# jac99/Egonn

Hardware: AMD Instinct MI355X
Metric: LiDAR scans/sec (descriptor extraction), 50k-pt clouds @ 0.1m voxel (higher is better)
Workload: dtype f32

## Files before the change

egonn_amd/_lib.py:

```python
from __future__ import annotations

import ctypes as C
import os
from typing import List, Optional, Sequence

import numpy as np
import torch

_HERE = os.path.dirname(os.path.abspath(__file__))
LIB_PATH = os.path.join(_HERE, "lib", "libegonn_hip.so")

QUANT_CARTESIAN, QUANT_POLAR = 0, 1
FLAG_DISABLE_GLOBAL, FLAG_DISABLE_LOCAL, FLAG_IGNORE_KP_REGRESSOR, FLAG_BF16 = 1, 2, 4, 8
FLAG_POOL_SPOC, FLAG_POOL_MAC = 16, 32
MINKFPN_SPLIT_TOPDOWN = 1
MINKFPN_BLOCKS = {'BasicBlock': 0, 'ECABasicBlock': 1}
MINKFPN_POOLING = {None: 0, 'GeM': 1, 'MAC': 2, 'SPoC': 3}

_P = C.c_void_p
_SIGS = [
    ("egonn_ctx_create", C.c_int, [C.POINTER(_P), C.c_int, C.c_int]),
    ("egonn_ctx_destroy", None, [_P]),
    ("egonn_last_error", C.c_char_p, []),
    ("egonn_debug_set_naive_conv", C.c_int, [_P, C.c_int]),
    ("egonn_debug_set_ksplit", C.c_int, [_P, C.c_int, C.c_int, C.c_int, C.c_int, C.c_int]),
    ("egonn_debug_set_resident", C.c_int, [_P, C.c_int, C.c_int]),
    ("egonn_debug_keep_level_features", C.c_int, [_P, C.c_int]),
    ("egonn_debug_set_trace", C.c_int, [_P]),
    ("egonn_prepare_maps", C.c_int, [_P, C.c_int, _P]),
    ("egonn_debug_rowgroup_tables", C.c_int, [_P, C.c_int, C.c_int, _P, _P, C.c_int64, C.POINTER(C.c_int64), _P]),
    ("egonn_debug_rowgroup_perm", C.c_int, [_P, C.c_int, C.c_int, _P, C.c_int64, C.POINTER(C.c_int64), _P]),
    ("egonn_debug_radix_sort_scratch_bytes", C.c_int64, [C.c_int64, C.c_int]),
    ("egonn_debug_radix_sort", C.c_int, [_P, _P, _P, _P, C.c_int64, C.c_int, _P, _P, C.c_int, C.c_int, C.c_int,
                                         C.POINTER(C.c_int32), _P, C.c_int64, _P]),
    ("egonn_debug_dense_group3", C.c_int, [_P, _P, _P, _P, _P, _P, _P]),
    ("egonn_debug_global_tail_scratch_bytes", C.c_int64, [C.c_int64]),
    ("egonn_debug_global_tail", C.c_int, [_P, _P, C.c_int, C.c_int64, _P, _P, _P, _P, _P, _P, C.c_int, C.c_int, _P, _P, _P, C.c_int64, _P]),
    ("egonn_voxelize", C.c_int, [_P, _P, C.POINTER(C.c_int64), C.c_int, C.c_int, C.POINTER(C.c_float), _P]),
    ("egonn_ctx_reserve", C.c_int, [_P, C.c_int64, C.c_int, C.POINTER(C.c_int64)]),
    ("egonn_voxelize_device", C.c_int, [_P, _P, C.c_int64, _P, C.c_int, C.c_int, C.POINTER(C.c_float), _P]),
    ("egonn_plan_status", C.c_int, [_P, _P]),
    ("egonn_ctx_set_exact_fp32", C.c_int, [_P, C.c_int]),
    ("egonn_ctx_set_operand_autoscale", C.c_int, [_P, C.c_int]),
    ("egonn_level_capacity", C.c_int, [_P, C.c_int, C.POINTER(C.c_int64)]),
    ("egonn_graph_begin", C.c_int, [_P]),
    ("egonn_graph_end", C.c_int, [_P, C.POINTER(_P)]),
    ("egonn_graph_launch", C.c_int, [_P, _P]),
    ("egonn_graph_destroy", None, [_P]),
    ("egonn_coords_set", C.c_int, [_P, _P, C.c_int64, C.c_int, _P]),
    ("egonn_level_count", C.c_int, [_P, C.c_int, C.POINTER(C.c_int64)]),
    ("egonn_level_batch_offsets", C.c_int, [_P, C.c_int, C.POINTER(C.c_int64)]),
    ("egonn_level_coords", C.c_int, [_P, C.c_int, _P, _P]),
    ("egonn_input_index", C.c_int, [_P, _P, _P]),
    ("egonn_conv", C.c_int, [_P, C.c_int, C.c_int, C.c_int, _P, C.c_int, _P, C.c_int, _P, _P, C.c_int, _P, _P]),
# ... 899 lines not shown
```

egonn_amd/csrc/coords.hip:

```cpp
#include "common.h"

#include <algorithm>
#include <stdarg.h>

namespace egonn {

static thread_local char g_err[1024] = "";
void set_error(const char* fmt, ...) {
  va_list ap;
  va_start(ap, fmt);
  vsnprintf(g_err, sizeof(g_err), fmt, ap);
  va_end(ap);
}
const char* last_error() { return g_err; }

const Switches& switches() {
  static const Switches sw = [] {
    auto on = [](const char* name) { return getenv(name) != nullptr; };
    auto num = [](const char* name, int unset) { const char* e = getenv(name); return e ? atoi(e) : unset; };
    const char* ds = getenv("EGONN_DEBUG_SYNC");
    return Switches{.debug_sync = ds && ds[0] == '1', .no_presplit = on("EGONN_NO_PRESPLIT"), .no_fused_down = on("EGONN_NO_FUSED_DOWN"),
                    .no_fused_lateral = on("EGONN_NO_FUSED_LATERAL"), .no_gated_k2s2 = on("EGONN_NO_GATED_K2S2"),
                    .no_fused_ghead = on("EGONN_NO_FUSED_GHEAD"), .no_fused_gtail = on("EGONN_NO_FUSED_GTAIL"),
                    .no_packed_laterals = on("EGONN_NO_PACKED_LATERALS"), .no_split_heads = on("EGONN_NO_SPLIT_HEADS"),
// ... 123 lines not shown
    vals[i] = (uint32_t)i;
  }
}

__global__ void coords_to_keys_kernel(const int32_t* __restrict__ c4, int64_t n, int cb, int Bmax,
                                      uint64_t* __restrict__ keys, uint32_t* __restrict__ vals,
                                      int32_t* __restrict__ flags) {
  const int64_t i = (int64_t)blockIdx.x * blockDim.x + threadIdx.x;
  if (i >= n) return;
  const int4 c = reinterpret_cast<const int4*>(c4)[i];
  uint64_t key;
  if (!encode_key(c.x, c.y, c.z, c.w, cb, key) || c.x >= Bmax) {
    atomicOr(flags, 1);
    key = ~0ull >> 1;
  }
  keys[i] = key;
  vals[i] = (uint32_t)i;
}

static constexpr int PYR_BLOCK = 256;
static constexpr int PYR_ROUNDS = 4;
static constexpr int PYR_TILE = PYR_BLOCK * PYR_ROUNDS;
static constexpr int NL = EGONN_MAX_LEVELS;

__device__ static inline int head_levels(const uint64_t* __restrict__ keys, int64_t i) {
  if (i == 0) return NL;
  const uint64_t d = keys[i] ^ keys[i - 1];
  if (d == 0) return 0;
  const int t = (63 - __clzll(d)) / 3;
  return (t >= NL - 1) ? NL : t + 1;
}

__device__ static inline int64_t clip_count(int64_t cap, const int64_t* __restrict__ n_dev) {
  if (!n_dev) return cap;
  const int64_t v = *n_dev;
  return v < cap ? v : cap;
}
__global__ __launch_bounds__(PYR_BLOCK) void pyramid_count_kernel(const uint64_t* __restrict__ keys, int64_t n_cap,
                                                                  const int64_t* __restrict__ n_dev,
                                                                  int32_t* __restrict__ tilecnt) {
  __shared__ int32_t cnt[PYR_BLOCK / 64][NL];
  const int64_t n = clip_count(n_cap, n_dev);
  const int tid = threadIdx.x, lane = tid & 63, wave = tid >> 6;
  const int64_t wbase = (int64_t)blockIdx.x * PYR_TILE + (int64_t)wave * 64 * PYR_ROUNDS;
  int32_t c[NL];
#pragma unroll
  for (int l = 0; l < NL; ++l) c[l] = 0;
  for (int r = 0; r < PYR_ROUNDS; ++r) {
    const int64_t i = wbase + r * 64 + lane;
    const int h = (i < n) ? head_levels(keys, i) : 0;
#pragma unroll
    for (int l = 0; l < NL; ++l) c[l] += __popcll(__ballot(h > l));
  }
  if (lane == 0) {
#pragma unroll
    for (int l = 0; l < NL; ++l) cnt[wave][l] = c[l];
  }
  __syncthreads();
  if (tid < NL) {
    int32_t s = 0;
    for (int w = 0; w < PYR_BLOCK / 64; ++w) s += cnt[w][tid];
    tilecnt[(int64_t)blockIdx.x * NL + tid] = s;
  }
}

struct PyramidOut {
  uint64_t* keys[NL];
  int32_t* parent[NL];
  int32_t* cstart[NL];
  int32_t* boff[EGONN_NUM_LEVELS];
  int32_t* perm0;
  int32_t* counts;
  int32_t* flags;
  int32_t cap[NL];
};

__global__ __launch_bounds__(PYR_BLOCK) void pyramid_apply_kernel(const uint64_t* __restrict__ keys,
                                                                  const uint32_t* __restrict__ vals, int64_t n_cap,
                                                                  const int64_t* __restrict__ n_dev,
                                                                  const int32_t* __restrict__ tilecnt, int ntiles,
                                                                  int cb, int B, PyramidOut out) {
  __shared__ int32_t red[PYR_BLOCK / 64][NL];
  const int64_t n = clip_count(n_cap, n_dev);
  __shared__ int32_t tilebase[NL];
  __shared__ int32_t wavecnt[PYR_BLOCK / 64][NL];
  const int tid = threadIdx.x, lane = tid & 63, wave = tid >> 6;
  const int tile = blockIdx.x;

  {
    int32_t p[NL];
#pragma unroll
    for (int l = 0; l < NL; ++l) p[l] = 0;
    for (int t = tid; t < tile; t += PYR_BLOCK) {
#pragma unroll
      for (int l = 0; l < NL; ++l) p[l] += tilecnt[(int64_t)t * NL + l];
    }
#pragma unroll
    for (int l = 0; l < NL; ++l) {
      int32_t v = p[l];
#pragma unroll
      for (int o = 32; o > 0; o >>= 1) v += __shfl_down(v, o, 64);
      if (lane == 0) red[wave][l] = v;
    }
    __syncthreads();
    if (tid < NL) {
      int32_t s = 0;
      for (int w = 0; w < PYR_BLOCK / 64; ++w) s += red[w][tid];
      tilebase[tid] = s;
    }
  }

  const int64_t wbase = (int64_t)tile * PYR_TILE + (int64_t)wave * 64 * PYR_ROUNDS;
  int hreg[PYR_ROUNDS];
  int32_t wc[NL];
#pragma unroll
  for (int l = 0; l < NL; ++l) wc[l] = 0;
#pragma unroll
  for (int r = 0; r < PYR_ROUNDS; ++r) {
    const int64_t i = wbase + r * 64 + lane;
    hreg[r] = (i < n) ? head_levels(keys, i) : 0;
#pragma unroll
    for (int l = 0; l < NL; ++l) wc[l] += __popcll(__ballot(hreg[r] > l));
  }
  if (lane == 0) {
#pragma unroll
    for (int l = 0; l < NL; ++l) wavecnt[wave][l] = wc[l];
  }
  __syncthreads();
  int32_t run[NL];
#pragma unroll
  for (int l = 0; l < NL; ++l) {
    int32_t s = tilebase[l];
    for (int w = 0; w < wave; ++w) s += wavecnt[w][l];
    run[l] = s;
  }

  const uint64_t lt = (lane == 0) ? 0ull : (~0ull >> (64 - lane));
  const int bshift = 3 * cb;
#pragma unroll
  for (int r = 0; r < PYR_ROUNDS; ++r) {
    const int64_t i = wbase + r * 64 + lane;
    const int h = hreg[r];
    const uint64_t key = (i < n) ? keys[i] : 0ull;
    int32_t excl[NL];
#pragma unroll
    for (int l = 0; l < NL; ++l) {
      const uint64_t m = __ballot(h > l);
      excl[l] = run[l] + __popcll(m & lt);
      run[l] += __popcll(m);
    }
    if (i < n && h > 0) {
      if (excl[0] < out.cap[0]) out.perm0[excl[0]] = (int32_t)vals[i];
#pragma unroll
      for (int l = 0; l < NL; ++l) {
        if (l < h && excl[l] < out.cap[l]) {
          out.keys[l][excl[l]] = key >> (3 * l);
          if (l >= 1) out.cstart[l][excl[l]] = min(excl[l - 1], out.cap[l - 1]);
          if (l + 1 < NL) {
            const int32_t g = (l + 1 < h) ? excl[l + 1] : excl[l + 1] - 1;
            out.parent[l][excl[l]] = min(g, out.cap[l + 1] - 1);
          }
        }
      }
      const int32_t b = (int32_t)(key >> bshift);
      const int32_t bprev = (i == 0) ? -1 : (int32_t)(keys[i - 1] >> bshift);
      if (b != bprev) {
        for (int32_t bb = bprev + 1; bb <= b && bb <= B; ++bb) {
#pragma unroll
          for (int l = 0; l < EGONN_NUM_LEVELS; ++l) out.boff[l][bb] = min(excl[l], out.cap[l]);
        }
      }
    }
    if (i == n - 1) {
      const int32_t blast = (int32_t)(key >> bshift);
#pragma unroll
      for (int l = 0; l < NL; ++l) {
        const int32_t total = excl[l] + (h > l ? 1 : 0);
        out.counts[l] = total;
        if (total > out.cap[l]) atomicOr(out.flags, 2);
        if (l >= 1) {
          const int32_t below = excl[l - 1] + (h > l - 1 ? 1 : 0);
          out.cstart[l][min(total, out.cap[l])] = min(below, out.cap[l - 1]);
        }
        if (l < EGONN_NUM_LEVELS) {
          for (int32_t bb = blast + 1; bb <= B; ++bb) out.boff[l][bb] = min(total, out.cap[l]);
        }
      }
      out.counts[NL] = blast + 1;
      out.counts[NL + 1] = (int32_t)n;
    }
  }
}

struct MaskArgs {
  const int32_t* cstartL[NL];
  const uint64_t* keys[NL];
  uint64_t* mask[NL];
  int32_t* bstart[NL];
  const int32_t* counts;
  int32_t prefix[NL + 1];
};

__device__ static inline int32_t level_rows(const int32_t* __restrict__ counts, int l, int32_t cap) {
  const int32_t v = counts[l];
  return v < cap ? v : cap;
}

__device__ static inline void block_mask_body(const MaskArgs& a, uint32_t vblock) {
  const int64_t t = (int64_t)vblock * 256 + threadIdx.x;
  if (t >= a.prefix[NL]) return;
  int L = 2;
  while (L < NL - 1 && t >= a.prefix[L + 1]) ++L;
  const int32_t j = (int32_t)(t - a.prefix[L]);
  if (j >= level_rows(a.counts, L, a.prefix[L + 1] - a.prefix[L])) return;
  const int32_t* cs1 = a.cstartL[L];
  const int32_t* cs2 = a.cstartL[L - 1];
  const int32_t s = cs2[cs1[j]];
  const int32_t e = cs2[cs1[j + 1]];
  const uint64_t* k = a.keys[L - 2];
  uint64_t m = 0;
  for (int32_t r = s; r < e; ++r) m |= 1ull << (k[r] & 63);
  a.mask[L][j] = m;
  a.bstart[L][j] = s;
}

__device__ static inline int32_t find_key(const uint64_t* __restrict__ keys, int32_t n, uint64_t q) {
  int32_t lo = 0, hi = n;
  while (lo < hi) {
    const int32_t mid = (lo + hi) >> 1;
    if (keys[mid] < q) lo = mid + 1; else hi = mid;
  }
  return (lo < n && keys[lo] == q) ? lo : -1;
}

__device__ static inline uint32_t bit_of_local(uint32_t lx, uint32_t ly, uint32_t lz) {
  return (lx & 1) | ((ly & 1) << 1) | ((lz & 1) << 2) | ((lx & 2) << 2) | ((ly & 2) << 3) | ((lz & 2) << 4);
}

__device__ static inline int32_t lookup_local(const uint64_t* nbm, const int32_t* nbs, int32_t nx, int32_t ny,
                                              int32_t nz) {
  const int32_t sx = (nx < 0) ? 0 : (nx > 3 ? 2 : 1);
  const int32_t sy = (ny < 0) ? 0 : (ny > 3 ? 2 : 1);
  const int32_t sz = (nz < 0) ? 0 : (nz > 3 ? 2 : 1);
  const int32_t slot = sx + 3 * sy + 9 * sz;
// ... 46 lines not shown
  const int32_t* badj;
  const uint64_t* bmask;
  const int32_t* bstart;
  int32_t* nbr;
  int32_t level, cap_blocks, cap_vox;
};
struct Blk27Args {
  const int32_t* badj;
  const uint64_t* bmask;
  const int32_t* bstart;
  int32_t cap2;
  uint64_t* t2m;
  int32_t* t2s;
};
struct Nbr27Pair {
  Nbr27Job job[2];
  const int32_t* counts;
  uint32_t split;
  uint32_t tail_at;
  Blk27Args blk;
};
__device__ static inline void blk27_body(const Blk27Args& b, const int32_t* __restrict__ counts, uint32_t vblock) {
  const int32_t t = (int32_t)(vblock * 256 + threadIdx.x);
  if (t >= level_rows(counts, 2, b.cap2) * 27) return;
  const int32_t a = b.badj[t];
  b.t2m[t] = a >= 0 ? b.bmask[a] : 0ull;
  b.t2s[t] = a >= 0 ? b.bstart[a] : 0;
}
__global__ __launch_bounds__(256) void nbr27_kernel(const Nbr27Pair a) {
  if (blockIdx.x >= a.tail_at) {
    blk27_body(a.blk, a.counts, blockIdx.x - a.tail_at);
    return;
  }
  const bool second = blockIdx.x >= a.split;
  const Nbr27Job& J = a.job[second ? 1 : 0];
  const uint64_t* __restrict__ vkeys = J.vkeys;
  const int32_t* __restrict__ badj = J.badj;
  const uint64_t* __restrict__ bmask = J.bmask;
  const int32_t* __restrict__ bstart = J.bstart;
  const int32_t* __restrict__ counts = a.counts;
  int32_t* __restrict__ nbr = J.nbr;
  const int level = J.level;
  const int32_t cap_blocks = J.cap_blocks, cap_vox = J.cap_vox;
  const uint32_t bid = second ? blockIdx.x - a.split : blockIdx.x;
  __shared__ uint64_t s_m[4][27];
  __shared__ int32_t s_s[4][27];
  const int lane = threadIdx.x & 63, wave = threadIdx.x >> 6;
  const int32_t j = (int32_t)bid * 4 + wave;
  const int32_t nblocks = level_rows(counts, level + 2, cap_blocks), nvox = level_rows(counts, level, cap_vox);
  if (j >= nblocks) return;
  const int32_t s = min(bstart[j], nvox);
  const int32_t e = min((j + 1 < nblocks) ? bstart[j + 1] : nvox, nvox);
  const int32_t idx = (lane < 27) ? badj[(int64_t)j * 27 + lane] : -1;
  const int32_t items = (e - s) * 27;
  uint64_t key0 = 0;
  if (lane < items) key0 = vkeys[s + lane / 27];
  if (lane < 27) {
    s_m[wave][lane] = idx >= 0 ? bmask[idx] : 0ull;
    s_s[wave][lane] = idx >= 0 ? bstart[idx] : 0;
  }
  __builtin_amdgcn_wave_barrier();
  __builtin_amdgcn_fence(__ATOMIC_ACQ_REL, "wavefront");
  for (int32_t t = lane; t < items; t += 64) {
    const int32_t v = t / 27, k = t - v * 27;
    const uint32_t lk = (uint32_t)((t == lane ? key0 : vkeys[s + v]) & 63);
    const int32_t lx = (lk & 1) | ((lk >> 2) & 2), ly = ((lk >> 1) & 1) | ((lk >> 3) & 2),
                  lz = ((lk >> 2) & 1) | ((lk >> 4) & 2);
    const int32_t nx = lx + (k % 3) - 1, ny = ly + (k / 3) % 3 - 1, nz = lz + k / 9 - 1;
    nbr[(int64_t)s * 27 + t] = lookup_local(s_m[wave], s_s[wave], nx, ny, nz);
  }
}

__global__ void count_valid_kernel(const int32_t* __restrict__ tbl, int64_t n, unsigned long long* __restrict__ out) {
  __shared__ int32_t red[4];
  int32_t c = 0;
  for (int64_t i = (int64_t)blockIdx.x * blockDim.x + threadIdx.x; i < n; i += (int64_t)gridDim.x * blockDim.x)
    c += (tbl[i] >= 0);
#pragma unroll
  for (int o = 32; o > 0; o >>= 1) c += __shfl_xor(c, o, 64);
  if ((threadIdx.x & 63) == 0) red[threadIdx.x >> 6] = c;
  __syncthreads();
  if (threadIdx.x == 0) atomicAdd(out, (unsigned long long)(red[0] + red[1] + red[2] + red[3]));
}
__global__ void count_k5_pairs_kernel(const uint64_t* __restrict__ vkeys, const int32_t* __restrict__ g0,
                                      const uint64_t* __restrict__ t2m, int32_t n, unsigned long long* __restrict__ out) {
  __shared__ int32_t red[4];
  int32_t c = 0;
  for (int32_t i = blockIdx.x * blockDim.x + threadIdx.x; i < n; i += gridDim.x * blockDim.x) {
    const uint32_t lk = (uint32_t)(vkeys[i] & 63);
    const int lx = (lk & 1) | ((lk >> 2) & 2), ly = ((lk >> 1) & 1) | ((lk >> 3) & 2), lz = ((lk >> 2) & 1) | ((lk >> 4) & 2);
    const uint64_t* m27 = t2m + (int64_t)g0[i] * 27;
    for (int k = 0; k < 125; ++k) {
// ... 42 lines not shown

__global__ void nbrT_kernel(const int32_t* __restrict__ parent, const uint64_t* __restrict__ keys,
                            const int32_t* __restrict__ counts, int32_t cap, int32_t* __restrict__ nbrT) {
  const int32_t c = blockIdx.x * blockDim.x + threadIdx.x;
  if (c >= level_rows(counts, 0, cap)) return;
  const int slot = (int)(keys[c] & 7);
  const int32_t p = parent[c];
  int32_t r[8];
#pragma unroll
  for (int q = 0; q < 8; ++q) r[q] = (q == slot) ? p : -1;
  int4* o = reinterpret_cast<int4*>(nbrT + (int64_t)c * 8);
  o[0] = make_int4(r[0], r[1], r[2], r[3]);
  o[1] = make_int4(r[4], r[5], r[6], r[7]);
}

struct Nbr8TArgs {
  const int32_t* cstart[EGONN_NUM_LEVELS];
  const uint64_t* ckeys[EGONN_NUM_LEVELS];
  const int32_t* parent[EGONN_NUM_LEVELS];
  const uint64_t* keys[EGONN_NUM_LEVELS];
  int32_t* nbr8[EGONN_NUM_LEVELS];
  int32_t* nbrT[EGONN_NUM_LEVELS];
  const int32_t* counts;
  int32_t prefix[EGONN_NUM_LEVELS + 1];
};
__device__ static inline void nbr8T_all_body(const Nbr8TArgs& a, uint32_t vblock) {
  const int64_t t = (int64_t)vblock * 256 + threadIdx.x;
  if (t >= a.prefix[EGONN_NUM_LEVELS]) return;
  int l = 1;
  while (l < EGONN_NUM_LEVELS - 1 && t >= a.prefix[l + 1]) ++l;
  const int32_t p = (int32_t)(t - a.prefix[l]);
  if (p >= level_rows(a.counts, l, a.prefix[l + 1] - a.prefix[l])) return;
  {
    int32_t r[8] = {-1, -1, -1, -1, -1, -1, -1, -1};
    const int32_t s = a.cstart[l][p], e = a.cstart[l][p + 1];
    const uint64_t* ck = a.ckeys[l];
    for (int32_t c = s; c < e; ++c) {
      const int slot = (int)(ck[c] & 7);
#pragma unroll
      for (int q = 0; q < 8; ++q)
        if (q == slot) r[q] = c;
    }
    int4* o = reinterpret_cast<int4*>(a.nbr8[l] + (int64_t)p * 8);
    o[0] = make_int4(r[0], r[1], r[2], r[3]);
    o[1] = make_int4(r[4], r[5], r[6], r[7]);
  }
  {
    const int slot = (int)(a.keys[l][p] & 7);
    const int32_t par = a.parent[l][p];
    int32_t r[8];
#pragma unroll
    for (int q = 0; q < 8; ++q) r[q] = (q == slot) ? par : -1;
    int4* o = reinterpret_cast<int4*>(a.nbrT[l] + (int64_t)p * 8);
    o[0] = make_int4(r[0], r[1], r[2], r[3]);
    o[1] = make_int4(r[4], r[5], r[6], r[7]);
  }
}

struct PlanTablesArgs {
  MaskArgs ma;
  Adj27Args adj;
  Adj27Args adj2;
  Nbr8TArgs na;
  const int32_t *parent0, *parent1;
  int32_t* g0;
  int32_t cap0;
  uint32_t b_mask, b_adj, b_adj2, b_gp, b_n8;
};
__global__ __launch_bounds__(256) void plan_tables_kernel(const PlanTablesArgs a) {
  uint32_t b = blockIdx.x;
  if (b < a.b_mask) { block_mask_body(a.ma, b); return; }
  b -= a.b_mask;
  if (b < a.b_adj) { adj27_search_body(a.adj, b); return; }
  b -= a.b_adj;
  if (b < a.b_adj2) { adj27_search_body(a.adj2, b); return; }
  b -= a.b_adj2;
  if (b < a.b_gp) {
    const int32_t i = (int32_t)(b * 256 + threadIdx.x);
    if (i < level_rows(a.ma.counts, 0, a.cap0)) a.g0[i] = a.parent1[a.parent0[i]];
    return;
  }
  b -= a.b_gp;
  nbr8T_all_body(a.na, b);
}

__global__ void decode_coords_kernel(const uint64_t* __restrict__ keys, int32_t n, int level, int cb,
                                     int32_t* __restrict__ out) {
  const int32_t i = blockIdx.x * blockDim.x + threadIdx.x;
  if (i >= n) return;
  const int cbL = cb - level;
  const uint64_t key = keys[i];
  const uint64_t mort = key & ((1ull << (3 * cbL)) - 1);
  const int32_t bias = 1 << (cb - 1);
  int4 o;
  o.x = (int32_t)(key >> (3 * cbL));
  o.y = ((int32_t)compact1by2(mort) << level) - bias;
  o.z = ((int32_t)compact1by2(mort >> 1) << level) - bias;
  o.w = ((int32_t)compact1by2(mort >> 2) << level) - bias;
  reinterpret_cast<int4*>(out)[i] = o;
}

static int batch_bits(int B) {
  int b = 0;
  while ((1 << b) < B) ++b;
  return b < 1 ? 1 : b;
}
// ... 98 lines not shown
  P.coord_bits = cb;
  P.n_input = n;
  P.cap_points = n;
  P.valid = true;
  P.exact = false;
  P.built_reserved = reserved;
  if (!reserved) {
    EGONN_TRY(plan_sync(ctx, stream));
    for (int l = 0; l < NL; ++l) P.cap[l] = P.lv[l].n;
  } else {
    for (int l = 0; l < NL; ++l) P.lv[l].n = P.cap[l];
  }
  P.valid = false;
  const int32_t* counts = ctx->dev_counts;

  PlanTablesArgs ta;
  MaskArgs& ma = ta.ma;
  int32_t pre = 0;
  for (int L = 0; L < NL; ++L) {
    ma.cstartL[L] = P.lv[L].cstart;
    ma.keys[L] = P.lv[L].keys;
    ma.mask[L] = nullptr;
    ma.bstart[L] = nullptr;
    ma.prefix[L] = 0;
  }
  ma.counts = counts;
  for (int L = 2; L < NL; ++L) {
    P.lv[L].mask = ma.mask[L] = A.alloc<uint64_t>(P.cap[L]);
    P.lv[L].bstart = ma.bstart[L] = A.alloc<int32_t>(P.cap[L]);
    EGONN_REQUIRE(ma.mask[L] && ma.bstart[L], EGONN_ERR_STATE, "plan arena too small");
    ma.prefix[L] = pre;
    pre += (int32_t)P.cap[L];
  }
  ma.prefix[NL] = pre;
  ta.b_mask = (unsigned)cdiv(pre, 256);
  for (int l = NL - 1; l >= 1; --l) {
    P.lv[l].nbr27 = A.alloc<int32_t>((size_t)P.cap[l] * 27);
    EGONN_REQUIRE(P.lv[l].nbr27, EGONN_ERR_STATE, "plan arena too small");
  }
  {
    Level& V = P.lv[NL - 2];
    Level& V1 = P.lv[NL - 1];
    const int32_t nv = (int32_t)P.cap[NL - 2], nv1 = (int32_t)P.cap[NL - 1];
    ta.adj = Adj27Args{V.keys, V1.keys, counts, NL - 2, NL - 1, cb - (NL - 2), cb - (NL - 1), nv, nv1, V.nbr27, V1.nbr27};
    ta.b_adj = (unsigned)cdiv(((int64_t)nv + nv1) * 27, 256);
  }
  const bool search67_ok = !switches().no_search67;
  const int search_from = (search67_ok && P.cap[NL - 4] <= 8192 && P.cap[NL - 3] <= 8192) ? NL - 4 : NL - 2;
  ta.b_adj2 = 0;
  ta.adj2 = ta.adj;
  if (search_from == NL - 4) {
    Level& V = P.lv[NL - 4];
    Level& V1 = P.lv[NL - 3];
    const int32_t nv = (int32_t)P.cap[NL - 4], nv1 = (int32_t)P.cap[NL - 3];
    ta.adj2 = Adj27Args{V.keys, V1.keys, counts, NL - 4, NL - 3, cb - (NL - 4), cb - (NL - 3), nv, nv1, V.nbr27, V1.nbr27};
    ta.b_adj2 = (unsigned)cdiv(((int64_t)nv + nv1) * 27, 256);
  }
  const int32_t n0 = (int32_t)P.cap[0], n2 = (int32_t)P.cap[2];
  {
    P.g0 = A.alloc<int32_t>(n0);
    P.t2m = A.alloc<uint64_t>((size_t)n2 * 27);
    P.t2s = A.alloc<int32_t>((size_t)n2 * 27);
    EGONN_REQUIRE(P.g0 && P.t2m && P.t2s, EGONN_ERR_STATE, "plan arena too small");
    ta.parent0 = P.lv[0].parent; ta.parent1 = P.lv[1].parent; ta.g0 = P.g0; ta.cap0 = n0;
    ta.b_gp = (unsigned)cdiv(n0, 256);
  }
  {
    Nbr8TArgs& na = ta.na;
    na.prefix[0] = na.prefix[1] = 0;
    na.counts = counts;
    for (int l = 1; l < EGONN_NUM_LEVELS; ++l) {
      Level& V = P.lv[l];
      const int32_t nv = (int32_t)P.cap[l];
      V.nbr8 = A.alloc<int32_t>((size_t)nv * 8);
      V.nbrT = A.alloc<int32_t>((size_t)nv * 8);
      EGONN_REQUIRE(V.nbr8 && V.nbrT, EGONN_ERR_STATE, "plan arena too small");
      na.cstart[l] = V.cstart;
      na.ckeys[l] = P.lv[l - 1].keys;
      na.parent[l] = V.parent;
      na.keys[l] = V.keys;
      na.nbr8[l] = V.nbr8;
      na.nbrT[l] = V.nbrT;
      na.prefix[l + 1] = na.prefix[l] + nv;
    }
    na.cstart[0] = nullptr; na.ckeys[0] = nullptr; na.parent[0] = nullptr; na.keys[0] = nullptr;
    na.nbr8[0] = nullptr; na.nbrT[0] = nullptr;
    ta.b_n8 = (unsigned)cdiv(na.prefix[EGONN_NUM_LEVELS], 256);
  }
  {
    const unsigned nb = ta.b_mask + ta.b_adj + ta.b_adj2 + ta.b_gp + ta.b_n8;
    if (nb > 0) hipLaunchKernelGGL(plan_tables_kernel, dim3(nb), dim3(256), 0, stream, ta);
  }

  Nbr27Pair pair;
  int npair = 0;
  pair.counts = counts;
  pair.split = 0;
  pair.tail_at = ~0u;
  pair.blk = Blk27Args{nullptr, nullptr, nullptr, 0, nullptr, nullptr};
  bool blk_done = false;
  auto flush = [&](bool last) {
    if (npair == 0 && !(last && !blk_done && n0 > 0)) return;
    if (npair == 1) pair.job[1] = pair.job[0];
    const unsigned g0 = npair >= 1 ? pair.split : 0u, g1 = npair == 2 ? (unsigned)cdiv(pair.job[1].cap_blocks, 4) : 0u;
    if (npair == 0) { pair.split = 0; pair.job[0] = Nbr27Job{nullptr, nullptr, nullptr, nullptr, nullptr, 1, 0, 0}; pair.job[1] = pair.job[0]; }
    unsigned extra = 0;
    pair.tail_at = ~0u;
    if (last && !blk_done && n0 > 0) {
      pair.tail_at = g0 + g1;
      pair.blk = Blk27Args{P.lv[2].nbr27, P.lv[2].mask, P.lv[2].bstart, n2, P.t2m, P.t2s};
// ... 170 lines not shown
    ctx->reserve_cap[l] = c;
  }
  ctx->reserve_points = max_points;
  ctx->reserve_batch = B;
  EGONN_TRY(ctx->plan_arena.ensure(plan_arena_bytes(max_points, B)));
  EGONN_TRY(ctx->sort_arena.ensure(std::max(radix_sort_scratch_bytes(max_points), radix_sort_segments_scratch_bytes(max_points, B))));
  ctx->reserved = true;
  return EGONN_OK;
}

int plan_level_coords(Ctx* ctx, int level, int32_t* out, hipStream_t stream) {
  EGONN_REQUIRE(ctx->plan.valid, EGONN_ERR_STATE, "no coordinate plan (call egonn_voxelize / egonn_coords_set first)");
  EGONN_REQUIRE(level >= 0 && level < EGONN_MAX_LEVELS, EGONN_ERR_INVALID, "level %d out of range", level);
  EGONN_TRY(plan_sync(ctx, stream));
  const Level& L = ctx->plan.lv[level];
  if (L.n == 0) return EGONN_OK;
  hipLaunchKernelGGL(decode_coords_kernel, dim3((unsigned)cdiv(L.n, 256)), dim3(256), 0, stream, L.keys, (int32_t)L.n,
                     level, ctx->plan.coord_bits, out);
  HIP_CHECK(hipGetLastError());
  return EGONN_OK;
}

}
```

include/egonn_hip.h:

```cpp
#ifndef EGONN_HIP_H
#define EGONN_HIP_H

#include <stdint.h>

#ifdef __cplusplus
extern "C" {
#endif

typedef struct egonn_ctx egonn_ctx;
typedef struct egonn_model egonn_model;

enum { EGONN_QUANT_CARTESIAN = 0, EGONN_QUANT_POLAR = 1 };
enum { EGONN_STATUS_OK = 0, EGONN_STATUS_INVALID = 1, EGONN_STATUS_HIP = 2, EGONN_STATUS_RANGE = 3, EGONN_STATUS_STATE = 4,
       EGONN_STATUS_CAPACITY = 5,
       EGONN_STATUS_FP16_RANGE = 6 };
enum { EGONN_FLAG_DISABLE_GLOBAL = 1, EGONN_FLAG_DISABLE_LOCAL = 2, EGONN_FLAG_IGNORE_KP_REGRESSOR = 4,
       EGONN_FLAG_BF16 = 8,
       EGONN_FLAG_POOL_SPOC = 16, EGONN_FLAG_POOL_MAC = 32 };

int egonn_ctx_create(egonn_ctx** ctx, int device, int coord_bits);
void egonn_ctx_destroy(egonn_ctx* ctx);
const char* egonn_last_error(void);
int egonn_debug_set_naive_conv(egonn_ctx* ctx, int on);
int egonn_debug_set_ksplit(egonn_ctx* ctx, int map_class, int level, int kparts, int kw, int col_parts);
int egonn_debug_set_resident(egonn_ctx* ctx, int mask, int max_workgroups);
int egonn_debug_keep_level_features(egonn_ctx* ctx, int on);
int egonn_debug_set_trace(void* device_buffer);
int egonn_debug_rowgroup_tables(egonn_ctx* ctx, int map_kind, int level_out, uint32_t* gmask_out, int32_t* snbr_out,
                                int64_t capacity_groups, int64_t* n_groups, void* stream);
int egonn_debug_rowgroup_perm(egonn_ctx* ctx, int map_kind, int level_out, int32_t* perm_out, int64_t capacity_groups,
                              int64_t* n_groups, void* stream);
int64_t egonn_debug_radix_sort_scratch_bytes(int64_t n, int n_segments);
int egonn_debug_radix_sort(uint64_t* keys_in, uint32_t* vals_in, uint64_t* keys_out, uint32_t* vals_out, int64_t n, int nbits,
                           const int64_t* n_dev, const int64_t* seg_offsets, int n_segments, int idx_bits, int either_pair,
                           int32_t* result_pair, void* scratch, int64_t scratch_bytes, void* stream);
int egonn_debug_dense_group3(const float* const in[3], const int64_t rows_capacity[3], const int32_t* const n_dev[3],
                             const float* const weight[3], const float* const packed[3], float* const out[3], void* stream);
int64_t egonn_debug_global_tail_scratch_bytes(int64_t rows_capacity);
int egonn_debug_global_tail(const float* g5, const int32_t* row_offsets, int batch_size, int64_t rows_capacity, const int32_t* n_dev,
                            const float* w0, const float* b0, const float* w1, const float* b1, const float* p, int pooling, int form,
                            float* partial, float* out, void* scratch, int64_t scratch_bytes, void* stream);

int egonn_voxelize(egonn_ctx* ctx, const float* points, const int64_t* scan_offsets, int batch_size, int quant_mode,
                   const float* step, void* stream);
int egonn_ctx_reserve(egonn_ctx* ctx, int64_t max_points, int batch_size, const int64_t* level_capacity);
int egonn_voxelize_device(egonn_ctx* ctx, const float* points, int64_t n_rows, const int64_t* scan_offsets_dev,
                          int batch_size, int quant_mode, const float* step, void* stream);
int egonn_plan_status(egonn_ctx* ctx, void* stream);
int egonn_ctx_set_exact_fp32(egonn_ctx* ctx, int on);
int egonn_ctx_set_operand_autoscale(egonn_ctx* ctx, int on);
int egonn_level_capacity(egonn_ctx* ctx, int level, int64_t* capacity);
typedef struct egonn_graph egonn_graph;
int egonn_graph_begin(void* stream);
int egonn_graph_end(void* stream, egonn_graph** graph);
// ... 351 lines not shown
```

Measured before the change: 23410.

## Hoist loads ahead of dependent work in coordinate-pyramid and plan-table kernels

The pyramid apply kernel now loads its keys and values into registers up front and gets each previous key through a wave shuffle rather than a second global read. It also packs the head levels into 4-bit fields. The mask, nbr8T, blk27, nbr27 and plan-table kernels clamp their indices so global loads can issue before the bounds checks, with sched barriers to keep that order. Level dispatch now uses per-level workgroup offsets instead of a linear prefix search, and child scans are unrolled in batches of 8 loads. New debug APIs expose the plan arena and its tables, and the clamped speculative loads read some redundant data.

```diff
diff --git a/egonn_amd/_lib.py b/egonn_amd/_lib.py
--- a/egonn_amd/_lib.py
+++ b/egonn_amd/_lib.py
@@ -30,6 +30,8 @@
     ("egonn_prepare_maps", C.c_int, [_P, C.c_int, _P]),
     ("egonn_debug_rowgroup_tables", C.c_int, [_P, C.c_int, C.c_int, _P, _P, C.c_int64, C.POINTER(C.c_int64), _P]),
     ("egonn_debug_rowgroup_perm", C.c_int, [_P, C.c_int, C.c_int, _P, C.c_int64, C.POINTER(C.c_int64), _P]),
+    ("egonn_debug_plan_arena", C.c_int, [_P, _P, C.c_int64, C.c_int, C.POINTER(C.c_int64)]),
+    ("egonn_debug_plan_tables", C.c_int, [_P, C.POINTER(C.c_int64), C.c_int, C.POINTER(C.c_int)]),
     ("egonn_debug_radix_sort_scratch_bytes", C.c_int64, [C.c_int64, C.c_int]),
     ("egonn_debug_radix_sort", C.c_int, [_P, _P, _P, _P, C.c_int64, C.c_int, _P, _P, C.c_int, C.c_int, C.c_int,
                                          C.POINTER(C.c_int32), _P, C.c_int64, _P]),
diff --git a/egonn_amd/csrc/coords.hip b/egonn_amd/csrc/coords.hip
--- a/egonn_amd/csrc/coords.hip
+++ b/egonn_amd/csrc/coords.hip
@@ -1,4 +1,4 @@
-#include "common.h"
+#include "model.h"
 
 #include <algorithm>
 #include <stdarg.h>
@@ -169,13 +169,17 @@
 static constexpr int PYR_ROUNDS = 4;
 static constexpr int PYR_TILE = PYR_BLOCK * PYR_ROUNDS;
 static constexpr int NL = EGONN_MAX_LEVELS;
-
-__device__ static inline int head_levels(const uint64_t* __restrict__ keys, int64_t i) {
-  if (i == 0) return NL;
-  const uint64_t d = keys[i] ^ keys[i - 1];
+static_assert(NL <= 15, "pyramid_apply_kernel packs a head level into 4 bits");
+
+__device__ static inline int head_levels_of(uint64_t key, uint64_t prev, bool first) {
+  if (first) return NL;
+  const uint64_t d = key ^ prev;
   if (d == 0) return 0;
   const int t = (63 - __clzll(d)) / 3;
   return (t >= NL - 1) ? NL : t + 1;
+}
+__device__ static inline int head_levels(const uint64_t* __restrict__ keys, int64_t i) {
+  return i == 0 ? NL : head_levels_of(keys[i], keys[i - 1], false);
 }
 
 __device__ static inline int64_t clip_count(int64_t cap, const int64_t* __restrict__ n_dev) {
@@ -183,6 +187,28 @@
   const int64_t v = *n_dev;
   return v < cap ? v : cap;
 }
+
+struct PyrKeys {
+  uint64_t key[PYR_ROUNDS];
+  uint64_t front;
+};
+__device__ static inline PyrKeys pyramid_load_keys(const uint64_t* __restrict__ keys, int64_t n_cap, int64_t wbase, int lane) {
+  PyrKeys k;
+  const int64_t last = n_cap - 1;
+#pragma unroll
+  for (int r = 0; r < PYR_ROUNDS; ++r) {
+    const int64_t i = wbase + r * 64 + lane;
+    k.key[r] = keys[i < last ? i : last];
+  }
+  const int64_t f = wbase - 1 < last ? wbase - 1 : last;
+  k.front = keys[f > 0 ? f : 0];
+  return k;
+}
+__device__ static inline uint64_t pyramid_prev_key(uint64_t key, uint64_t carry, int lane) {
+  const uint64_t up = __shfl_up(key, 1, 64);
+  return lane == 0 ? carry : up;
+}
+
 __global__ __launch_bounds__(PYR_BLOCK) void pyramid_count_kernel(const uint64_t* __restrict__ keys, int64_t n_cap,
                                                                   const int64_t* __restrict__ n_dev,
                                                                   int32_t* __restrict__ tilecnt) {
@@ -228,11 +254,20 @@
                                                                   const int32_t* __restrict__ tilecnt, int ntiles,
                                                                   int cb, int B, PyramidOut out) {
   __shared__ int32_t red[PYR_BLOCK / 64][NL];
-  const int64_t n = clip_count(n_cap, n_dev);
   __shared__ int32_t tilebase[NL];
   __shared__ int32_t wavecnt[PYR_BLOCK / 64][NL];
   const int tid = threadIdx.x, lane = tid & 63, wave = tid >> 6;
   const int tile = blockIdx.x;
+  const int64_t wbase = (int64_t)tile * PYR_TILE + (int64_t)wave * 64 * PYR_ROUNDS;
+  const PyrKeys k = pyramid_load_keys(keys, n_cap, wbase, lane);
+  uint32_t val[PYR_ROUNDS];
+#pragma unroll
+  for (int r = 0; r < PYR_ROUNDS; ++r) {
+    const int64_t i = wbase + r * 64 + lane;
+    val[r] = vals[i < n_cap - 1 ? i : n_cap - 1];
+  }
+  const int64_t n = clip_count(n_cap, n_dev);
+  __builtin_amdgcn_sched_barrier(0);
 
   {
     int32_t p[NL];
@@ -257,17 +292,21 @@
     }
   }
 
-  const int64_t wbase = (int64_t)tile * PYR_TILE + (int64_t)wave * 64 * PYR_ROUNDS;
-  int hreg[PYR_ROUNDS];
+  const int bshift = 3 * cb;
+  uint32_t hpack = 0;
   int32_t wc[NL];
 #pragma unroll
   for (int l = 0; l < NL; ++l) wc[l] = 0;
+  uint64_t carry = k.front;
 #pragma unroll
   for (int r = 0; r < PYR_ROUNDS; ++r) {
     const int64_t i = wbase + r * 64 + lane;
-    hreg[r] = (i < n) ? head_levels(keys, i) : 0;
-#pragma unroll
-    for (int l = 0; l < NL; ++l) wc[l] += __popcll(__ballot(hreg[r] > l));
+    const uint64_t prev = pyramid_prev_key(k.key[r], carry, lane);
+    carry = __shfl(k.key[r], 63, 64);
+    const int h = (i < n) ? head_levels_of(k.key[r], prev, i == 0) : 0;
+    hpack |= (uint32_t)h << (4 * r);
+#pragma unroll
+    for (int l = 0; l < NL; ++l) wc[l] += __popcll(__ballot(h > l));
   }
   if (lane == 0) {
 #pragma unroll
@@ -283,12 +322,14 @@
   }
 
   const uint64_t lt = (lane == 0) ? 0ull : (~0ull >> (64 - lane));
-  const int bshift = 3 * cb;
+  carry = k.front;
 #pragma unroll
   for (int r = 0; r < PYR_ROUNDS; ++r) {
     const int64_t i = wbase + r * 64 + lane;
-    const int h = hreg[r];
-    const uint64_t key = (i < n) ? keys[i] : 0ull;
+    const int h = (int)((hpack >> (4 * r)) & 15u);
+    const uint64_t key = (i < n) ? k.key[r] : 0ull;
+    const uint64_t prev = pyramid_prev_key(k.key[r], carry, lane);
+    carry = __shfl(k.key[r], 63, 64);
     int32_t excl[NL];
 #pragma unroll
     for (int l = 0; l < NL; ++l) {
@@ -297,7 +338,7 @@
       run[l] += __popcll(m);
     }
     if (i < n && h > 0) {
-      if (excl[0] < out.cap[0]) out.perm0[excl[0]] = (int32_t)vals[i];
+      if (excl[0] < out.cap[0]) out.perm0[excl[0]] = (int32_t)val[r];
 #pragma unroll
       for (int l = 0; l < NL; ++l) {
         if (l < h && excl[l] < out.cap[l]) {
@@ -310,7 +351,7 @@
         }
       }
       const int32_t b = (int32_t)(key >> bshift);
-      const int32_t bprev = (i == 0) ? -1 : (int32_t)(keys[i - 1] >> bshift);
+      const int32_t bprev = (i == 0) ? -1 : (int32_t)(prev >> bshift);
       if (b != bprev) {
         for (int32_t bb = bprev + 1; bb <= b && bb <= B; ++bb) {
 #pragma unroll
@@ -345,7 +386,8 @@
   uint64_t* mask[NL];
   int32_t* bstart[NL];
   const int32_t* counts;
-  int32_t prefix[NL + 1];
+  int32_t wg[NL + 1];
+  int32_t cap[NL];
 };
 
 __device__ static inline int32_t level_rows(const int32_t* __restrict__ counts, int l, int32_t cap) {
@@ -354,19 +396,31 @@
 }
 
 __device__ static inline void block_mask_body(const MaskArgs& a, uint32_t vblock) {
-  const int64_t t = (int64_t)vblock * 256 + threadIdx.x;
-  if (t >= a.prefix[NL]) return;
   int L = 2;
-  while (L < NL - 1 && t >= a.prefix[L + 1]) ++L;
-  const int32_t j = (int32_t)(t - a.prefix[L]);
-  if (j >= level_rows(a.counts, L, a.prefix[L + 1] - a.prefix[L])) return;
+#pragma unroll
+  for (int q = 3; q < NL; ++q) L += (int32_t)vblock >= a.wg[q];
+  const int32_t cap = a.cap[L];
+  const int32_t j = (int32_t)(vblock - a.wg[L]) * 256 + threadIdx.x;
+  const int32_t jc = min(j, cap - 1);
   const int32_t* cs1 = a.cstartL[L];
   const int32_t* cs2 = a.cstartL[L - 1];
-  const int32_t s = cs2[cs1[j]];
-  const int32_t e = cs2[cs1[j + 1]];
+  const int32_t c0 = cs1[jc], c1 = cs1[jc + 1];
+  const int32_t rows = level_rows(a.counts, L, cap);
+  __builtin_amdgcn_sched_barrier(0);
+  if (j >= rows) return;
+  const int32_t s = cs2[c0];
+  const int32_t e = cs2[c1];
+  __builtin_amdgcn_sched_barrier(0);
   const uint64_t* k = a.keys[L - 2];
   uint64_t m = 0;
-  for (int32_t r = s; r < e; ++r) m |= 1ull << (k[r] & 63);
+  for (int32_t r0 = s; r0 < e; r0 += 8) {
+    uint64_t kk[8];
+#pragma unroll
+    for (int c = 0; c < 8; ++c) kk[c] = k[min(r0 + c, e - 1)];
+    __builtin_amdgcn_sched_barrier(0);
+#pragma unroll
+    for (int c = 0; c < 8; ++c) m |= (r0 + c < e) ? 1ull << (kk[c] & 63) : 0ull;
+  }
   a.mask[L][j] = m;
   a.bstart[L][j] = s;
 }
@@ -459,10 +513,15 @@
 };
 __device__ static inline void blk27_body(const Blk27Args& b, const int32_t* __restrict__ counts, uint32_t vblock) {
   const int32_t t = (int32_t)(vblock * 256 + threadIdx.x);
-  if (t >= level_rows(counts, 2, b.cap2) * 27) return;
-  const int32_t a = b.badj[t];
-  b.t2m[t] = a >= 0 ? b.bmask[a] : 0ull;
-  b.t2s[t] = a >= 0 ? b.bstart[a] : 0;
+  const int32_t a = b.badj[min(t, b.cap2 * 27 - 1)];
+  const int32_t n2 = level_rows(counts, 2, b.cap2);
+  __builtin_amdgcn_sched_barrier(0);
+  if (t >= n2 * 27) return;
+  const int32_t ac = max(a, 0);
+  const uint64_t m = b.bmask[ac];
+  const int32_t s = b.bstart[ac];
+  b.t2m[t] = a >= 0 ? m : 0ull;
+  b.t2s[t] = a >= 0 ? s : 0;
 }
 __global__ __launch_bounds__(256) void nbr27_kernel(const Nbr27Pair a) {
   if (blockIdx.x >= a.tail_at) {
@@ -482,29 +541,43 @@
   const uint32_t bid = second ? blockIdx.x - a.split : blockIdx.x;
   __shared__ uint64_t s_m[4][27];
   __shared__ int32_t s_s[4][27];
-  const int lane = threadIdx.x & 63, wave = threadIdx.x >> 6;
+  __shared__ uint32_t s_k[4][64];
+  const int lane = threadIdx.x & 63, wave = __builtin_amdgcn_readfirstlane(threadIdx.x >> 6);
   const int32_t j = (int32_t)bid * 4 + wave;
   const int32_t nblocks = level_rows(counts, level + 2, cap_blocks), nvox = level_rows(counts, level, cap_vox);
-  if (j >= nblocks) return;
-  const int32_t s = min(bstart[j], nvox);
-  const int32_t e = min((j + 1 < nblocks) ? bstart[j + 1] : nvox, nvox);
-  const int32_t idx = (lane < 27) ? badj[(int64_t)j * 27 + lane] : -1;
-  const int32_t items = (e - s) * 27;
-  uint64_t key0 = 0;
-  if (lane < items) key0 = vkeys[s + lane / 27];
+  if (j >= nblocks || nvox <= 0) return;
+  const int32_t bs0 = bstart[j], bs1 = bstart[min(j + 1, nblocks - 1)];
+  const int32_t idx = badj[(int64_t)j * 27 + min(lane, 26)];
+  __builtin_amdgcn_sched_barrier(0);
+  const int32_t s = min(bs0, nvox);
+  const int32_t e = min((j + 1 < nblocks) ? bs1 : nvox, nvox);
+  const int32_t nv = e - s;
+  const int32_t idc = max(idx, 0);
+  const uint64_t nm = bmask[idc];
+  const int32_t ns = bstart[idc];
+  const uint64_t key = vkeys[min(s + lane, nvox - 1)];
+  __builtin_amdgcn_sched_barrier(0);
   if (lane < 27) {
-    s_m[wave][lane] = idx >= 0 ? bmask[idx] : 0ull;
-    s_s[wave][lane] = idx >= 0 ? bstart[idx] : 0;
-  }
-  __builtin_amdgcn_wave_barrier();
-  __builtin_amdgcn_fence(__ATOMIC_ACQ_REL, "wavefront");
-  for (int32_t t = lane; t < items; t += 64) {
-    const int32_t v = t / 27, k = t - v * 27;
-    const uint32_t lk = (uint32_t)((t == lane ? key0 : vkeys[s + v]) & 63);
-    const int32_t lx = (lk & 1) | ((lk >> 2) & 2), ly = ((lk >> 1) & 1) | ((lk >> 3) & 2),
-                  lz = ((lk >> 2) & 1) | ((lk >> 4) & 2);
-    const int32_t nx = lx + (k % 3) - 1, ny = ly + (k / 3) % 3 - 1, nz = lz + k / 9 - 1;
-    nbr[(int64_t)s * 27 + t] = lookup_local(s_m[wave], s_s[wave], nx, ny, nz);
+    s_m[wave][lane] = idx >= 0 ? nm : 0ull;
+    s_s[wave][lane] = idx >= 0 ? ns : 0;
+  }
+  s_k[wave][lane] = (uint32_t)key & 63u;
+  for (int32_t vb = 0; vb < nv; vb += 64) {
+    if (vb > 0) {
+      __builtin_amdgcn_wave_barrier();
+      s_k[wave][lane] = (uint32_t)vkeys[min(s + vb + lane, nvox - 1)] & 63u;
+    }
+    __builtin_amdgcn_wave_barrier();
+    __builtin_amdgcn_fence(__ATOMIC_ACQ_REL, "wavefront");
+    const int32_t items = min(nv - vb, 64) * 27;
+    for (int32_t t = lane; t < items; t += 64) {
+      const int32_t v = t / 27, k = t - v * 27;
+      const uint32_t lk = s_k[wave][v];
+      const int32_t lx = (lk & 1) | ((lk >> 2) & 2), ly = ((lk >> 1) & 1) | ((lk >> 3) & 2),
+                    lz = ((lk >> 2) & 1) | ((lk >> 4) & 2);
+      const int32_t nx = lx + (k % 3) - 1, ny = ly + (k / 3) % 3 - 1, nz = lz + k / 9 - 1;
+      nbr[((int64_t)s + vb) * 27 + t] = lookup_local(s_m[wave], s_s[wave], nx, ny, nz);
+    }
   }
 }
 
@@ -593,32 +666,44 @@
   int32_t* nbr8[EGONN_NUM_LEVELS];
   int32_t* nbrT[EGONN_NUM_LEVELS];
   const int32_t* counts;
-  int32_t prefix[EGONN_NUM_LEVELS + 1];
+  int32_t wg[EGONN_NUM_LEVELS + 1];
+  int32_t cap[EGONN_NUM_LEVELS];
 };
 __device__ static inline void nbr8T_all_body(const Nbr8TArgs& a, uint32_t vblock) {
-  const int64_t t = (int64_t)vblock * 256 + threadIdx.x;
-  if (t >= a.prefix[EGONN_NUM_LEVELS]) return;
   int l = 1;
-  while (l < EGONN_NUM_LEVELS - 1 && t >= a.prefix[l + 1]) ++l;
-  const int32_t p = (int32_t)(t - a.prefix[l]);
-  if (p >= level_rows(a.counts, l, a.prefix[l + 1] - a.prefix[l])) return;
+#pragma unroll
+  for (int q = 2; q < EGONN_NUM_LEVELS; ++q) l += (int32_t)vblock >= a.wg[q];
+  const int32_t cap = a.cap[l];
+  const int32_t p = (int32_t)(vblock - a.wg[l]) * 256 + threadIdx.x;
+  const int32_t pc = min(p, cap - 1);
+  const int32_t s = a.cstart[l][pc], e = a.cstart[l][pc + 1];
+  const uint64_t key = a.keys[l][pc];
+  const int32_t par = a.parent[l][pc];
+  const int32_t rows = level_rows(a.counts, l, cap);
+  __builtin_amdgcn_sched_barrier(0);
+  if (p >= rows) return;
   {
     int32_t r[8] = {-1, -1, -1, -1, -1, -1, -1, -1};
-    const int32_t s = a.cstart[l][p], e = a.cstart[l][p + 1];
     const uint64_t* ck = a.ckeys[l];
-    for (int32_t c = s; c < e; ++c) {
-      const int slot = (int)(ck[c] & 7);
-#pragma unroll
-      for (int q = 0; q < 8; ++q)
-        if (q == slot) r[q] = c;
+    for (int32_t c0 = s; c0 < e; c0 += 8) {
+      uint64_t kk[8];
+#pragma unroll
+      for (int c = 0; c < 8; ++c) kk[c] = ck[min(c0 + c, e - 1)];
+      __builtin_amdgcn_sched_barrier(0);
+#pragma unroll
+      for (int c = 0; c < 8; ++c) {
+        const int slot = (c0 + c < e) ? (int)(kk[c] & 7) : -1;
+#pragma unroll
+        for (int q = 0; q < 8; ++q)
+          if (q == slot) r[q] = c0 + c;
+      }
     }
     int4* o = reinterpret_cast<int4*>(a.nbr8[l] + (int64_t)p * 8);
     o[0] = make_int4(r[0], r[1], r[2], r[3]);
     o[1] = make_int4(r[4], r[5], r[6], r[7]);
   }
   {
-    const int slot = (int)(a.keys[l][p] & 7);
-    const int32_t par = a.parent[l][p];
+    const int slot = (int)(key & 7);
     int32_t r[8];
 #pragma unroll
     for (int q = 0; q < 8; ++q) r[q] = (q == slot) ? par : -1;
@@ -639,20 +724,22 @@
   uint32_t b_mask, b_adj, b_adj2, b_gp, b_n8;
 };
 __global__ __launch_bounds__(256) void plan_tables_kernel(const PlanTablesArgs a) {
-  uint32_t b = blockIdx.x;
-  if (b < a.b_mask) { block_mask_body(a.ma, b); return; }
-  b -= a.b_mask;
-  if (b < a.b_adj) { adj27_search_body(a.adj, b); return; }
-  b -= a.b_adj;
-  if (b < a.b_adj2) { adj27_search_body(a.adj2, b); return; }
-  b -= a.b_adj2;
-  if (b < a.b_gp) {
+  const uint32_t e0 = a.b_mask, e1 = e0 + a.b_adj, e2 = e1 + a.b_adj2, e3 = e2 + a.b_gp;
+  const uint32_t bx = blockIdx.x;
+  const int part = (bx >= e0) + (bx >= e1) + (bx >= e2) + (bx >= e3);
+  if (part == 0) { block_mask_body(a.ma, bx); return; }
+  if (part == 1) { adj27_search_body(a.adj, bx - e0); return; }
+  if (part == 2) { adj27_search_body(a.adj2, bx - e1); return; }
+  if (part == 3) {
+    const uint32_t b = bx - e2;
     const int32_t i = (int32_t)(b * 256 + threadIdx.x);
-    if (i < level_rows(a.ma.counts, 0, a.cap0)) a.g0[i] = a.parent1[a.parent0[i]];
+    const int32_t p0 = a.parent0[min(i, a.cap0 - 1)];
+    const int32_t rows = level_rows(a.ma.counts, 0, a.cap0);
+    __builtin_amdgcn_sched_barrier(0);
+    if (i < rows) a.g0[i] = a.parent1[p0];
     return;
   }
-  b -= a.b_gp;
-  nbr8T_all_body(a.na, b);
+  nbr8T_all_body(a.na, bx - e3);
 }
 
 __global__ void decode_coords_kernel(const uint64_t* __restrict__ keys, int32_t n, int level, int cb,
@@ -797,18 +884,20 @@
     ma.keys[L] = P.lv[L].keys;
     ma.mask[L] = nullptr;
     ma.bstart[L] = nullptr;
-    ma.prefix[L] = 0;
+    ma.wg[L] = 0;
+    ma.cap[L] = 0;
   }
   ma.counts = counts;
   for (int L = 2; L < NL; ++L) {
     P.lv[L].mask = ma.mask[L] = A.alloc<uint64_t>(P.cap[L]);
     P.lv[L].bstart = ma.bstart[L] = A.alloc<int32_t>(P.cap[L]);
     EGONN_REQUIRE(ma.mask[L] && ma.bstart[L], EGONN_ERR_STATE, "plan arena too small");
-    ma.prefix[L] = pre;
-    pre += (int32_t)P.cap[L];
-  }
-  ma.prefix[NL] = pre;
-  ta.b_mask = (unsigned)cdiv(pre, 256);
+    ma.wg[L] = pre;
+    ma.cap[L] = (int32_t)P.cap[L];
+    pre += (int32_t)cdiv(P.cap[L], 256);
+  }
+  ma.wg[NL] = pre;
+  ta.b_mask = (unsigned)pre;
   for (int l = NL - 1; l >= 1; --l) {
     P.lv[l].nbr27 = A.alloc<int32_t>((size_t)P.cap[l] * 27);
     EGONN_REQUIRE(P.lv[l].nbr27, EGONN_ERR_STATE, "plan arena too small");
@@ -842,7 +931,8 @@
   }
   {
     Nbr8TArgs& na = ta.na;
-    na.prefix[0] = na.prefix[1] = 0;
+    na.wg[0] = na.wg[1] = 0;
+    na.cap[0] = 0;
     na.counts = counts;
     for (int l = 1; l < EGONN_NUM_LEVELS; ++l) {
       Level& V = P.lv[l];
@@ -856,11 +946,12 @@
       na.keys[l] = V.keys;
       na.nbr8[l] = V.nbr8;
       na.nbrT[l] = V.nbrT;
-      na.prefix[l + 1] = na.prefix[l] + nv;
+      na.cap[l] = nv;
+      na.wg[l + 1] = na.wg[l] + (int32_t)cdiv(nv, 256);
     }
     na.cstart[0] = nullptr; na.ckeys[0] = nullptr; na.parent[0] = nullptr; na.keys[0] = nullptr;
     na.nbr8[0] = nullptr; na.nbrT[0] = nullptr;
-    ta.b_n8 = (unsigned)cdiv(na.prefix[EGONN_NUM_LEVELS], 256);
+    ta.b_n8 = (unsigned)na.wg[EGONN_NUM_LEVELS];
   }
   {
     const unsigned nb = ta.b_mask + ta.b_adj + ta.b_adj2 + ta.b_gp + ta.b_n8;
@@ -1077,3 +1168,52 @@
 }
 
 }
+
+API int egonn_debug_plan_arena(egonn_ctx* c, void* buf, int64_t bytes, int to_arena, int64_t* arena_bytes) {
+  EGONN_REQUIRE(c && arena_bytes, EGONN_ERR_INVALID, "debug_plan_arena: null argument");
+  HIP_CHECK(hipSetDevice(c->device));
+  const egonn::Arena& A = c->plan_arena;
+  *arena_bytes = (int64_t)A.cap;
+  if (!buf) return EGONN_OK;
+  EGONN_REQUIRE(A.base && bytes >= 0 && (size_t)bytes <= A.cap, EGONN_ERR_INVALID, "debug_plan_arena: %lld bytes, the arena holds %zu",
+                (long long)bytes, A.cap);
+  HIP_CHECK(hipDeviceSynchronize());
+  HIP_CHECK(to_arena ? hipMemcpy(A.base, buf, (size_t)bytes, hipMemcpyDeviceToDevice)
+                     : hipMemcpy(buf, A.base, (size_t)bytes, hipMemcpyDeviceToDevice));
+  HIP_CHECK(hipDeviceSynchronize());
+  return EGONN_OK;
+}
+API int egonn_debug_plan_tables(egonn_ctx* c, int64_t* out, int max_entries, int* n_entries) {
+  using namespace egonn;
+  EGONN_REQUIRE(c && out && n_entries, EGONN_ERR_INVALID, "debug_plan_tables: null argument");
+  REQUIRE_PLAN(c);
+  const Plan& P = c->plan;
+  const char* base = c->plan_arena.base;
+  const int64_t n = P.cap_points;
+  int e = 0;
+  bool full = false;
+  auto put = [&](int table, int level, const void* ptr, int64_t bytes) {
+    if (!ptr) return;
+    if (e >= max_entries) { full = true; return; }
+    out[4 * e + 0] = table; out[4 * e + 1] = level; out[4 * e + 2] = (const char*)ptr - base; out[4 * e + 3] = bytes;
+    ++e;
+  };
+  for (int l = 0; l < NL; ++l) {
+    const Level& V = P.lv[l];
+    put(0, l, V.keys, n * 8); put(1, l, V.parent, n * 4); put(2, l, V.cstart, (n + 1) * 4);
+    put(3, l, V.mask, P.cap[l] * 8); put(4, l, V.bstart, P.cap[l] * 4); put(5, l, V.nbr27, P.cap[l] * 108);
+    put(6, l, V.nbr8, P.cap[l] * 32); put(7, l, V.nbrT, P.cap[l] * 32);
+    const RowGroups* rg[3] = {&V.rg27, &V.rg8, &V.rgT};
+    for (int m = 0; m < 3; ++m) {
+      if (!rg[m]->built) continue;
+      const int64_t G = rg[m]->cap_groups;
+      put(13 + 5 * m, l, rg[m]->perm, G * 64); put(14 + 5 * m, l, rg[m]->snbr, G * rg[m]->K * 64); put(15 + 5 * m, l, rg[m]->gmask, G * 4);
+      put(16 + 5 * m, l, rg[m]->meta, ((int64_t)P.batch + 2) * 4); put(17 + 5 * m, l, rg[m]->order4, (G / 4 + 16) * 4);
+    }
+  }
+  put(8, 0, P.perm0, n * 4); put(9, 0, P.g0, P.cap[0] * 4); put(10, 2, P.t2m, P.cap[2] * 216); put(11, 2, P.t2s, P.cap[2] * 108);
+  put(12, 0, P.lv[0].boff, (int64_t)EGONN_NUM_LEVELS * (P.batch + 1) * 4);
+  EGONN_REQUIRE(!full, EGONN_ERR_INVALID, "debug_plan_tables: more than %d tables", max_entries);
+  *n_entries = e;
+  return EGONN_OK;
+}
diff --git a/include/egonn_hip.h b/include/egonn_hip.h
--- a/include/egonn_hip.h
+++ b/include/egonn_hip.h
@@ -30,6 +30,8 @@
                                 int64_t capacity_groups, int64_t* n_groups, void* stream);
 int egonn_debug_rowgroup_perm(egonn_ctx* ctx, int map_kind, int level_out, int32_t* perm_out, int64_t capacity_groups,
                               int64_t* n_groups, void* stream);
+int egonn_debug_plan_arena(egonn_ctx* ctx, void* device_buf, int64_t bytes, int to_arena, int64_t* arena_bytes);
+int egonn_debug_plan_tables(egonn_ctx* ctx, int64_t* out, int max_entries, int* n_entries);
 int64_t egonn_debug_radix_sort_scratch_bytes(int64_t n, int n_segments);
 int egonn_debug_radix_sort(uint64_t* keys_in, uint32_t* vals_in, uint64_t* keys_out, uint32_t* vals_out, int64_t n, int nbits,
                            const int64_t* n_dev, const int64_t* seg_offsets, int n_segments, int idx_bits, int either_pair,
```

Result: no change. 23450 (median of 2 runs) (+0.2%).
